# Haochen-Wang409/U2PL

Hardware: AMD Instinct MI355X
Metric: train images/sec at 769x769 (R101-DeepLabv3+) (higher is better)
Workload: dtype f32

## Files before the change

### include/u2pl_hip.h

```cpp
#ifndef U2PL_HIP_H
#define U2PL_HIP_H

#include <stddef.h>
#include <stdint.h>

#ifdef __cplusplus
extern "C" {
#endif

#ifndef __HIP_PLATFORM_AMD__
typedef struct ihipStream_t* hipStream_t;
#endif

#define U2PL_SEL_MAX_SLOTS 8
#define U2PL_SEL_WORD_NVALID 0
#define U2PL_SEL_WORD_NTOTAL 1
#define U2PL_SEL_WORD_VAL 40
#define U2PL_SEL_WORD_THR 56

int u2pl_bilinear_up_f32(const float* in, long sn, long sc, long sh, long sw, int N, int C, int h, int w,
                         float* out_nchw, int H, int W, hipStream_t stream);
int u2pl_bilinear_up_bwd_f32(const float* gout_nchw, int N, int C, int H, int W, float* gin, long sn, long sc,
                             long sh, long sw, int h, int w, hipStream_t stream);
int u2pl_pseudo_label_f32(const float* logits_nchw, int N, int C, int H, int W, float* conf, long long* label,
                          hipStream_t stream);
int u2pl_entropy_f32(const float* logits_nchw, const long long* label, int ignore, int N, int C, int H, int W,
                     float* entropy, unsigned* ws, hipStream_t stream);
int u2pl_entropy_up_f32(const float* in, long sn, long sc, long sh, long sw, int N, int C, int h, int w, int H, int W,
                        const long long* label, int ignore, float* entropy, unsigned* ws, hipStream_t stream);
size_t u2pl_select_workspace_bytes(void);
int u2pl_select_f32(const float* values, long n, int nspec, const int* spec_kind_dev, const float* q32_dev,
                    const long long* kparam_dev, const float* fparam_dev, unsigned* ws, int hist0_done,
                    hipStream_t stream);
int u2pl_apply_drop_i64(const float* entropy, const unsigned* thr_bits, long long* target, int ignore, long n,
                        unsigned* nkept, hipStream_t stream);
int u2pl_reliability_masks(const float* entropy, const unsigned* thr_lo_bits, const unsigned* thr_hi_bits,
                           const long long* label_l, const long long* label_u, int ignore, int B, int H, int W,
                           int h, int w, int negative_high_entropy, float* low_mask, float* high_mask,
                           unsigned* lbits, hipStream_t stream);
int u2pl_reliability_apply(const float* entropy, const unsigned* thr_bits, const long long* label_l,
                           const long long* label_u, int ignore, int B, int H, int W, int h, int w,
                           int negative_high_entropy, long long* target_u, unsigned* nkept, float* low_mask,
                           float* high_mask, unsigned* lbits, hipStream_t stream);
int u2pl_pack_class_bits(const long long* onehot, int N, int C, int h, int w, unsigned* bits, hipStream_t stream);
int u2pl_unpack_class_bits(const unsigned* bits, int N, int C, int h, int w, long long* onehot,
                           hipStream_t stream);

int u2pl_contra_classify(const float* prob, long sn, long sc, long sp, const unsigned* lbits,
                         const float* low_mask, const float* high_mask, int N2, int num_labeled, int C, int h,
                         int w, float thr_p, float thr_n, int low_rank, int high_rank, unsigned* abits,
                         unsigned* lowbits, unsigned* nbits, void* compact_workspace, hipStream_t stream);
size_t u2pl_compact_workspace_bytes(long P);
int u2pl_compact_lists(const unsigned* abits, const unsigned* lowbits, const unsigned* nbits, long P, int C,
                       void* workspace, int* idx, long cap, unsigned* counts, int counted, hipStream_t stream);
size_t u2pl_proto_workspace_bytes(long P, int C, int D);
int u2pl_class_prototypes(const float* rows, long ld, int D, const int* idx, long cap, const unsigned* counts,
                          int C, long P, void* workspace, float* proto, const unsigned* lowbits,
                          hipStream_t stream);
size_t u2pl_contra_phase1_workspace_bytes(long P, int C, int D);
int u2pl_contra_phase1(const float* prob, long sn, long sc, long sp, const unsigned* lbits, const float* low_mask,
                       const float* high_mask, int N2, int num_labeled, int C, int h, int w, float thr_p, float thr_n,
                       int low_rank, int high_rank, const float* rows, long ld, int D, unsigned* abits, unsigned* lowbits,
                       unsigned* nbits, int* idx, long cap, unsigned* counts, float* proto, void* workspace,
                       hipStream_t stream);
int u2pl_gather_rows_f32(const float* rows, long ld, int D, const int* list, long n, float* out,
                         hipStream_t stream);
size_t u2pl_bank_state_bytes(int C);
int u2pl_bank_init(long long* state, int C, const long long* caps_host, hipStream_t stream);
int u2pl_bank_enqueue_f32(long long* state, float* storage, int D, const float* rows, long ld, const int* idx,
                          long idx_stride, const long long* row_start_dev, const unsigned* counts_dev, int C,
                          hipStream_t stream);
int u2pl_bank_append_f32(float* bank, long cap, long tail, int D, const float* rows, long ld, const int* list,
                         long n_new, hipStream_t stream);
int u2pl_bank_append_multi_f32(const long long* desc_dev, int nclass, int D, long ld, long max_new,
                               hipStream_t stream);
size_t u2pl_infonce_job_bytes(void);
int u2pl_infonce_f32(const void* jobs_dev, int njobs, const float* rep, long ld, int D, int Q, int K,
                     float temp, float* loss_q, float* ganchor, int* anchor_pix, int* head, int* next,
                     const int* seg_len, hipStream_t stream);
size_t u2pl_infonce_fused_workspace_bytes(int njobs, int Q);
int u2pl_infonce_fused_f32(const void* jobs_dev, int njobs, const float* rep, long ld, int D, int Q, int K, float temp,
                           float* loss_q, float* ganchor, int* anchor_pix, int* head, int* next, const int* seg_len,
                           float* zero_dst, long zero_ld, const int* zero_pix, long zero_n, void* workspace,
                           float inv_valid_seg, float* loss, hipStream_t stream);
int u2pl_infonce_reduce_f32(const float* loss_q, int njobs, int Q, float inv_valid_seg, float* loss,
                            hipStream_t stream);
int u2pl_scatter_rows_ordered_f32(float* dst, long ld, int D, const int* pix, const int* next, int* head,
                                  const int* order, const int* seg_pos, const int* seg_len, const float* src, long n,
                                  const float* gout_dev, float scale, hipStream_t stream);
int u2pl_zero_rows_f32(float* dst, long ld, int D, const int* pix, long n, hipStream_t stream);

size_t u2pl_ce_workspace_bytes(void);
int u2pl_ce_fwd_f32(const float* logits_nchw, const long long* target, int ignore, int N, int C, int H, int W,
                    int unsup_weight, void* workspace, float* out3, hipStream_t stream);
int u2pl_ce_bwd_f32(const float* logits_nchw, const long long* target, int ignore, int N, int C, int H, int W,
                    const float* out3_dev, const float* gout_dev, float gmul, float* grad, hipStream_t stream);
int u2pl_ce_fwd_weighted_f32(const float* logits_nchw, const long long* target, int ignore, int N, int C, int H, int W,
                             const float* class_weight, void* workspace, float* out3, hipStream_t stream);
int u2pl_ce_bwd_weighted_f32(const float* logits_nchw, const long long* target, int ignore, int N, int C, int H, int W,
                             const float* class_weight, const float* out3_dev, const float* gout_dev, float gmul,
                             float* grad, hipStream_t stream);
int u2pl_ohem_prob_f32(const float* logits_nchw, const long long* target, int ignore, int N, int C, int H,
                       int W, float* mask_prob, unsigned* ws, hipStream_t stream);
int u2pl_ohem_apply_i64(const float* mask_prob, const unsigned* thr_bits, const long long* target, int ignore,
                        long n, long long* kept_target, hipStream_t stream);
int u2pl_confusion_hist_f32(const float* logits_nchw, const long long* target, int ignore, int N, int C, int H, int W,
                            long long* hist3c, hipStream_t stream);

int u2pl_predict_map_f32(const float* in, long sn, long sc, long sh, long sw, int N, int C, int h, int w, int H, int W,
                         unsigned char* label, const unsigned char* palette, unsigned char* rgb, hipStream_t stream);
int u2pl_infer_input_u8_f32(const unsigned char* img_hwc, int h, int w, const float* lut, float* out_hwc, int H, int W,
                            hipStream_t stream);
int u2pl_window_fuse_f32(float* pred, float* count, int C, int H, int W, const float* in, long sc, long sh, long sw, int h,
                         int w, int h0, int w0, int hc, int wc, int flip, int softmax, float weight, int bump,
                         hipStream_t stream);
int u2pl_predict_entropy_f32(const float* in, long sn, long sc, long sh, long sw, int N, int C, int h, int w, int H, int W,
                             int prob, unsigned char* label, float* entropy, hipStream_t stream);
int u2pl_reliable_map_u8(unsigned char* label, const float* entropy, const unsigned* thr_bits, long n,
                         const unsigned char* palette, unsigned char* rgb, unsigned char* heat, float heat_scale,
                         unsigned* ndropped, hipStream_t stream);
int u2pl_lut_u8(const unsigned char* in, unsigned char* out, long n, const unsigned char* lut256, hipStream_t stream);

int u2pl_conv2d_fwd_f32(const float* x, long ldx, const float* w, const float* bias, float* y, long ldy, int N,
                        int Hin, int Win, int Cin, int Hout, int Wout, int Cout, int R, int S, int stride,
                        int pad, int dil, hipStream_t stream);
int u2pl_conv2d_fwd_stat_blocks(int N, int Hout, int Wout, int Cout);
int u2pl_conv2d_fwd_bnstats_f32(const float* x, long ldx, const float* w, const float* bias, float* y, long ldy,
                                int N, int Hin, int Win, int Cin, int Hout, int Wout, int Cout, int R, int S,
                                int stride, int pad, int dil, const float* pivot, float* stats_partial,
                                hipStream_t stream);
int u2pl_colreduce_finish_f32(const float* partial, int nblk, int C, double* sums, hipStream_t stream);
int u2pl_conv2d_fwd_bnact_f32(const float* x, long ldx, const float* w, const float* bias, float* y, long ldy, int N,
                              int Hin, int Win, int Cin, int Hout, int Wout, int Cout, int R, int S, int stride,
                              int pad, int dil, const float* mean, const float* invstd, const float* gamma,
                              const float* beta, const float* res, long ldr, int relu, hipStream_t stream);
int u2pl_gemm_batched_f32(const float* x, long ldx, long zx, const float* w, long zw, float* y, long ldy, long zy,
                          long M, int K, int Nn, int batch, hipStream_t stream);
size_t u2pl_wino_tiles(int N, int H, int W, int dil, int mt);
int u2pl_wino_stat_blocks(long tiles, int O);
int u2pl_wino_input_f32(const float* x, long ldx, int N, int H, int W, int C, int dil, int mt, float* V,
                        hipStream_t stream);
int u2pl_wino_weight_f32(const float* w, int O, int C, int transposed, int mt, float* U, hipStream_t stream);
int u2pl_wino_gy_f32(const float* gy, long ldg, int N, int H, int W, int O, int dil, int mt, float* Mg,
                     hipStream_t stream);
int u2pl_wgrad_batched_splits(long M, int Cin, int Cout, int batch);
size_t u2pl_wgrad_batched_workspace_bytes(long M, int Cin, int Cout, int batch);
int u2pl_wgrad_batched_f32(const float* dy, long lddy, long zdy, const float* x, long ldx, long zx, float* part,
                           long M, int Cin, int Cout, int batch, hipStream_t stream);
int u2pl_wino_wgrad_finish_f32(const float* part, int nsplit, int O, int C, int mt, int accumulate, float* dw,
                               hipStream_t stream);
int u2pl_wino_output_f32(const float* Mb, int N, int H, int W, int O, int dil, int mt, const float* bias, float* y,
                         long ldy, float* stats_partial, const float* pivot, hipStream_t stream);
int u2pl_wino_output_bnact_f32(const float* Mb, int N, int H, int W, int O, int dil, int mt, const float* bias, float* y,
                               long ldy, const float* mean, const float* invstd, const float* gamma, const float* beta,
                               const float* res, long ldr, int relu, hipStream_t stream);
int u2pl_conv2d_fwd_bf16op_f32(const float* x, long ldx, const float* w, const float* bias, float* y, long ldy, int N,
                               int Hin, int Win, int Cin, int Hout, int Wout, int Cout, int R, int S, int stride,
                               int pad, int dil, hipStream_t stream);
int u2pl_conv2d_fwd_bnstats_bf16op_f32(const float* x, long ldx, const float* w, const float* bias, float* y, long ldy,
                                       int N, int Hin, int Win, int Cin, int Hout, int Wout, int Cout, int R, int S,
                                       int stride, int pad, int dil, const float* pivot, float* stats_partial,
                                       hipStream_t stream);
int u2pl_conv2d_dgrad_bf16op_f32(const float* dy, long lddy, const float* wT, float* dx, long lddx, int N, int Hin,
                                 int Win, int Cin, int Hout, int Wout, int Cout, int R, int S, int stride, int pad,
                                 int dil, hipStream_t stream);
int u2pl_conv2d_wgrad_bf16op_f32(const float* dy, long lddy, const float* x, long ldx, float* dw, void* workspace,
                                 int accumulate, int N, int Hin, int Win, int Cin, int Hout, int Wout, int Cout, int R,
                                 int S, int stride, int pad, int dil, hipStream_t stream);
int u2pl_conv2d_dgrad_f32(const float* dy, long lddy, const float* wT, float* dx, long lddx, int N, int Hin,
                          int Win, int Cin, int Hout, int Wout, int Cout, int R, int S, int stride, int pad,
                          int dil, hipStream_t stream);
int u2pl_weight_transpose_f32(const float* w, float* wt, int Cout, int RS, int Cin, hipStream_t stream);
size_t u2pl_conv2d_wgrad_workspace_bytes(int N, int Hout, int Wout, int Cin, int Cout, int R, int S);
int u2pl_conv2d_wgrad_f32(const float* dy, long lddy, const float* x, long ldx, float* dw, void* workspace,
                          int accumulate, int N, int Hin, int Win, int Cin, int Hout, int Wout, int Cout, int R,
                          int S, int stride, int pad, int dil, hipStream_t stream);
int u2pl_wgrad_set_tr(int on);
int u2pl_im2col_f32(const float* x, long ldx, float* col, int Kp, int N, int Hin, int Win, int Cin, int Hout,
                    int Wout, int R, int S, int stride, int pad, int dil, hipStream_t stream);

int u2pl_gconv2d_fwd_f32(const float* x, long ldx, const float* w, const float* bias, float* y, long ldy, int N, int Hin,
                         int Win, int Cin, int Hout, int Wout, int Cout, int R, int S, int stride, int pad, int dil,
                         int groups, hipStream_t stream);
int u2pl_gconv2d_dgrad_f32(const float* dy, long lddy, const float* w, float* dx, long lddx, int N, int Hin, int Win,
                           int Cin, int Hout, int Wout, int Cout, int R, int S, int stride, int pad, int dil, int groups,
                           hipStream_t stream);
size_t u2pl_gconv2d_wgrad_workspace_bytes(int N, int Hout, int Wout, int Cin, int Cout, int R, int S, int groups);
int u2pl_gconv2d_wgrad_f32(const float* dy, long lddy, const float* x, long ldx, float* dw, void* workspace,
                           int accumulate, int N, int Hin, int Win, int Cin, int Hout, int Wout, int Cout, int R,
                           int S, int stride, int pad, int dil, int groups, hipStream_t stream);

int u2pl_dwconv2d_fwd_f32(const float* x, long ldx, const float* w, const float* bias, float* y, long ldy, int N, int Hin,
                          int Win, int Cin, int Hout, int Wout, int Cout, int R, int S, int stride, int pad, int dil,
                          int groups, hipStream_t stream);
int u2pl_dwconv2d_dgrad_f32(const float* dy, long lddy, const float* w, float* dx, long lddx, int N, int Hin, int Win,
                            int Cin, int Hout, int Wout, int Cout, int R, int S, int stride, int pad, int dil, int groups,
                            hipStream_t stream);
size_t u2pl_dwconv2d_wgrad_workspace_bytes(int N, int Hout, int Wout, int Cin, int Cout, int R, int S, int groups);
int u2pl_dwconv2d_wgrad_f32(const float* dy, long lddy, const float* x, long ldx, float* dw, void* workspace,
                            int accumulate, int N, int Hin, int Win, int Cin, int Hout, int Wout, int Cout, int R,
                            int S, int stride, int pad, int dil, int groups, hipStream_t stream);

size_t u2pl_weight_split3_bytes(int rows, int K, int batch);
int u2pl_weight_split3_f32(const float* w, long zw, int rows, int K, int batch, void* out, hipStream_t stream);
int u2pl_weight_split3_multi_f32(const void* jobs, int njobs, long total, hipStream_t stream);
int u2pl_weight_split3_pad_rows(int rows);
int u2pl_wino_weight_multi_f32(const void* jobs, int njobs, long total, hipStream_t stream);
size_t u2pl_weight_split2h_bytes(int rows, int K, int batch);
int u2pl_weight_split2h_f32(const float* w, long zw, int rows, int K, int batch, void* out, hipStream_t stream);
int u2pl_weight_rebuild2h_job_bytes(void);
int u2pl_weight_rebuild2h_span(int which);
int u2pl_weight_rebuild2h_f32(const void* jobs, int n_flat, int n_wino, long seg_total, long amax_total, int wino_mblocks,
                              int wino_pblocks, hipStream_t stream);
int u2pl_amax_words(void);
int u2pl_absmax_f32(const float* x, long ld, long M, int C, float* out, int clear, hipStream_t stream);

int u2pl_igemm_ws_stat_blocks(int N, int Hout, int Wout);
int u2pl_igemm_ws_set_persist(int on);
int u2pl_conv2d_fwd_ws_f32(const float* x, long ldx, const void* wsplit, const float* bias, float* y, long ldy, int N,
                           int Hin, int Win, int Cin, int Hout, int Wout, int Cout, int R, int S, int stride, int pad,
                           int dil, hipStream_t stream);
int u2pl_conv2d_fwd_bnstats_ws_f32(const float* x, long ldx, const void* wsplit, const float* bias, float* y, long ldy,
                                   int N, int Hin, int Win, int Cin, int Hout, int Wout, int Cout, int R, int S,
                                   int stride, int pad, int dil, const float* pivot, float* stats_partial,
                                   hipStream_t stream);
int u2pl_conv2d_fwd_bnact_ws_f32(const float* x, long ldx, const void* wsplit, const float* bias, float* y, long ldy, int N,
                                 int Hin, int Win, int Cin, int Hout, int Wout, int Cout, int R, int S, int stride,
                                 int pad, int dil, const float* mean, const float* invstd, const float* gamma,
                                 const float* beta, const float* res, long ldr, int relu, hipStream_t stream);
int u2pl_conv2d_dgrad_ws_f32(const float* dy, long lddy, const void* wTsplit, float* dx, long lddx, int N, int Hin,
                             int Win, int Cin, int Hout, int Wout, int Cout, int R, int S, int stride, int pad, int dil,
                             hipStream_t stream);
int u2pl_gemm_batched_ws_f32(const float* x, long ldx, long zx, const void* wsplit, float* y, long ldy, long zy, long M,
                             int K, int Nn, int batch, hipStream_t stream);

int u2pl_bn_apply_amax_f32(const float* x, long ldx, const float* mean, const float* invstd, const float* gamma, const float* beta,
                           const float* res, long ldr, int relu, const float* drop, long rows_per_image, float* y, long ldy, long M,
                           int C, float* y_amax, hipStream_t stream);
int u2pl_bn_bwd_apply_amax_f32(const float* dy, long lddy, const float* x, long ldx, const float* y, long ldy, const float* mean,
                               const float* invstd, const float* gamma, const float* drop, long rows_per_image, const double* sums,
                               double count, float* dx, long lddx, float* dres, long lddr, long M, int C, const double* psums,
                               float* gsink, float* bsink, int accumulate, float* dx_amax, float* dres_amax, const float* relu_beta,
                               hipStream_t stream);
int u2pl_bn_bwd_sums_mx_f32(const float* dy, long lddy, const float* x, long ldx, const float* mean, const float* invstd,
                            const float* gamma, const float* beta, const float* drop, long rows_per_image, long M, int C,
                            void* workspace, double* sums, hipStream_t stream);
int u2pl_bn_apply_bits_f32(const float* x, long ldx, const float* mean, const float* invstd, const float* gamma, const float* beta,
                           const float* res, long ldr, int relu, const float* drop, long rows_per_image, float* y, long ldy, long M,
                           int C, float* y_amax, unsigned* bits, long ldb, hipStream_t stream);
int u2pl_bn_bwd_sums_bits_f32(const float* dy, long lddy, const float* x, long ldx, const unsigned* bits, long ldb,
                              const float* mean, const float* invstd, const float* drop, long rows_per_image, long M, int C,
                              void* workspace, double* sums, hipStream_t stream);
int u2pl_bn_bwd_apply_bits_f32(const float* dy, long lddy, const float* x, long ldx, const unsigned* bits, long ldb,
                               const float* mean, const float* invstd, const float* gamma, const float* drop, long rows_per_image,
                               const double* sums, double count, float* dx, long lddx, float* dres, long lddr, long M, int C,
                               const double* psums, float* gsink, float* bsink, int accumulate, float* dx_amax, float* dres_amax,
                               hipStream_t stream);
int u2pl_wino_input_amax_f32(const float* x, long ldx, int N, int H, int W, int C, int dil, int mt, float* V, float* v_amax,
                             hipStream_t stream);
int u2pl_wino_output_bnact_amax_f32(const float* Mb, int N, int H, int W, int O, int dil, int mt, const float* bias, float* y,
                                    long ldy, const float* mean, const float* invstd, const float* gamma, const float* beta,
                                    const float* res, long ldr, int relu, float* y_amax, hipStream_t stream);
int u2pl_wino_gy_amax_f32(const float* gy, long ldg, int N, int H, int W, int O, int dil, int mt, float* Mg, float* mg_amax,
                          hipStream_t stream);
int u2pl_conv2d_fwd_wsh_f32(const float* x, long ldx, const float* x_amax, const void* wsplit, const float* bias, float* y, long ldy,
                            int N, int Hin, int Win, int Cin, int Hout, int Wout, int Cout, int R, int S, int stride, int pad,
                            int dil, hipStream_t stream);
int u2pl_conv2d_fwd_bnstats_wsh_f32(const float* x, long ldx, const float* x_amax, const void* wsplit, const float* bias, float* y,
                                    long ldy, int N, int Hin, int Win, int Cin, int Hout, int Wout, int Cout, int R, int S,
                                    int stride, int pad, int dil, const float* pivot, float* stats_partial, hipStream_t stream);
int u2pl_conv2d_fwd_bnact_wsh_f32(const float* x, long ldx, const float* x_amax, const void* wsplit, const float* bias, float* y,
                                  long ldy, int N, int Hin, int Win, int Cin, int Hout, int Wout, int Cout, int R, int S,
                                  int stride, int pad, int dil, const float* mean, const float* invstd, const float* gamma,
                                  const float* beta, const float* res, long ldr, int relu, float* y_amax, hipStream_t stream);
int u2pl_conv2d_dgrad_wsh_f32(const float* dy, long lddy, const float* dy_amax, const void* wTsplit, float* dx, long lddx, int N,
                              int Hin, int Win, int Cin, int Hout, int Wout, int Cout, int R, int S, int stride, int pad, int dil,
                              hipStream_t stream);
int u2pl_gemm_batched_wsh_f32(const float* x, long ldx, long zx, const float* x_amax, const void* wsplit, float* y, long ldy, long zy,
                              long M, int K, int Nn, int batch, hipStream_t stream);
int u2pl_wgrad_h_eligible(int Cin, int Cout);
int u2pl_conv2d_wgrad_h_f32(const float* dy, long lddy, const float* dy_amax, const float* x, long ldx, const float* x_amax, float* dw,
                            void* workspace, int accumulate, int N, int Hin, int Win, int Cin, int Hout, int Wout, int Cout, int R,
                            int S, int stride, int pad, int dil, hipStream_t stream);
int u2pl_wgrad_batched_h_f32(const float* dy, long lddy, long zdy, const float* dy_amax, const float* x, long ldx, long zx,
                             const float* x_amax, float* part, long M, int Cin, int Cout, int batch, hipStream_t stream);

size_t u2pl_colreduce_workspace_bytes(long Mseg, int nseg, int C);
int u2pl_bn_stats_f32(const float* x, long ld, long M, int C, const float* pivot, void* workspace, double* sums,
                      hipStream_t stream);
int u2pl_colsum_f32(const float* x, long ld, long Mseg, int nseg, int C, void* workspace, double* sums,
                    hipStream_t stream);
int u2pl_bn_bwd_sums_f32(const float* dy, long lddy, const float* x, long ldx, const float* y, long ldy,
                         const float* mean, const float* invstd, const float* drop, long rows_per_image, long M,
                         int C, void* workspace, double* sums, hipStream_t stream);
int u2pl_bn_finalize_f32(const double* sums, double count, const float* pivot, int C, float eps, float momentum,
                         float* mean, float* invstd, float* running_mean, float* running_var, hipStream_t stream);
int u2pl_bn_eval_invstd_f32(const float* running_var, int C, float eps, float* invstd, hipStream_t stream);
int u2pl_bn_finish_finalize_f32(const float* partial, int nblk, int C, double count, const float* pivot, float eps,
                                float momentum, float* mean, float* invstd, float* running_mean, float* running_var,
                                double* sums_out, hipStream_t stream);
size_t u2pl_bn_eval_invstd_job_bytes(void);
int u2pl_bn_eval_invstd_multi_f32(const void* jobs_dev, int njobs, long total, hipStream_t stream);
int u2pl_bn_apply_f32(const float* x, long ldx, const float* mean, const float* invstd, const float* gamma,
                      const float* beta, const float* res, long ldr, int relu, const float* drop,
                      long rows_per_image, float* y, long ldy, long M, int C, hipStream_t stream);
int u2pl_bn_bwd_apply_f32(const float* dy, long lddy, const float* x, long ldx, const float* y, long ldy,
                          const float* mean, const float* invstd, const float* gamma, const float* drop,
                          long rows_per_image, const double* sums, double count, float* dx, long lddx, float* dres,
                          long lddr, long M, int C, hipStream_t stream);
int u2pl_bn_bwd_apply_pg_f32(const float* dy, long lddy, const float* x, long ldx, const float* y, long ldy,
                             const float* mean, const float* invstd, const float* gamma, const float* drop,
                             long rows_per_image, const double* sums, double count, float* dx, long lddx, float* dres,
                             long lddr, long M, int C, const double* psums, float* gsink, float* bsink, int accumulate,
                             hipStream_t stream);
int u2pl_sums_to_f32(const double* sums, int n, float scale, int accumulate, float* out, hipStream_t stream);
int u2pl_maxpool3s2_fwd_f32(const float* x, long ldx, int N, int H, int W, int C, int Ho, int Wo, float* y, long ldy,
                            unsigned char* tap, hipStream_t stream);
int u2pl_maxpool3s2_bwd_f32(const float* dy, long lddy, const unsigned char* tap, int N, int H, int W, int C, int Ho,
                            int Wo, float* dx, long lddx, hipStream_t stream);
int u2pl_copy_rows_f32(const float* src, long lds, float* dst, long ldd, long M, int C, int accumulate,
                       hipStream_t stream);
int u2pl_copy_cols_f32(const float* src, long lds, float* dst, long ldd, long M, int C, hipStream_t stream);
int u2pl_broadcast_rows_f32(const float* v, long ldv, float scale, float* dst, long ldd, long rows_per_image, long M,
                            int C, hipStream_t stream);
int u2pl_bilinear_rows_fwd_f32(const float* x, long ldx, int N, int h, int w, int C, int H, int W, float* y, long ldy,
                               hipStream_t stream);
int u2pl_bilinear_rows_bwd_f32(const float* dy, long lddy, int N, int h, int w, int C, int H, int W, float* dx,
                               long lddx, hipStream_t stream);
int u2pl_softmax_rows_f32(const float* x, long ldx, float* y, long ldy, long M, int C, hipStream_t stream);
int u2pl_sgd_step_f32(float* p, const float* g, float* buf, long n, long b1, long b2, float lr0, float lr1, float lr2,
                      float momentum, float weight_decay, int first, float grad_scale, hipStream_t stream);
int u2pl_ema_update_f32(float* t, const float* s, long n, float decay, float one_minus_decay, hipStream_t stream);
int u2pl_adam_step_f32(float* p, const float* g, float* exp_avg, float* exp_avg_sq, long n, long b1, long b2, float lr0,
                       float lr1, float lr2, float beta1, float one_minus_beta1, float beta2, float one_minus_beta2,
                       float eps, float weight_decay, float bias_correction1, float bias_correction2_sqrt,
                       float grad_scale, hipStream_t stream);
size_t u2pl_kernel_launches(void);
int u2pl_conv_set_split(int on);
int u2pl_conv_get_split(void);
int u2pl_debug_phase1_times(unsigned* buf);
size_t u2pl_reliability_fused_workspace_bytes(int G);
size_t u2pl_reliability_fused_cand_floats(long n_px, int G);
int u2pl_reliability_fused(const float* logits_low, long sn, long sc, long sh, long sw, int B, int C, int h, int w,
                           int H, int W, const long long* label_u, const long long* label_l, int ignore, int nspec,
                           const float* q32_host, int negative_high_entropy, int hm, int wm, float* entropy,
                           long long* target_u, float* low_mask, float* high_mask, unsigned* lbits,
                           unsigned* workspace, float* cand, int G, unsigned epoch, int flags, hipStream_t stream);
int u2pl_cutmix_f32(const float* img, const long long* label, const float* conf, const int* boxes_dev, int B, int C,
                    int H, int W, float* out_img, long long* out_label, float* out_conf, hipStream_t stream);

int u2pl_dense_small_f32(const float* x, long ldx, const float* w, const float* bias, float* y, long ldy, int M, int K,
                         int Cout, hipStream_t stream);
int u2pl_strong_aug_f32(const float* img, const long long* label, const float* conf, const int* boxes_dev,
                        const unsigned long long* sel_dev, int mode, int B, int C, int H, int W, float* out_img,
                        long long* out_label, float* out_conf, hipStream_t stream);
int u2pl_label_presence_i64(const long long* label, int B, long HW, unsigned long long* bits, hipStream_t stream);

int u2pl_window_accumulate_f32(float* pred, float* count, int C, int H, int W, const float* src, int h0, int w0,
                               int hc, int wc, hipStream_t stream);
int u2pl_window_normalize_f32(float* pred, const float* count, int C, int H, int W, hipStream_t stream);

int u2pl_augment_u8_f32(const unsigned char* img, const unsigned char* lab, const int* params, int B, int H, int W,
                        int Sh, int Sw, const float* mean3, const float* std3, float* out_img, long long* out_lab,
                        hipStream_t stream);

#define U2PL_AUG_REC 16
#define U2PL_AUG_ROTATE 1
#define U2PL_AUG_BLUR 2
size_t u2pl_augment_ex_scratch_bytes(int B, int Sh, int Sw, int mode);
int u2pl_augment_ex_u8_f32(const unsigned char* img, const unsigned char* lab, const long long* offsets,
                           const int* records, int B, int H, int W, int Sh, int Sw, int ignore_label, int mode,
                           const float* mean3, const float* std3, const float* blur_w, float* scratch, float* out_img,
                           long long* out_lab, hipStream_t stream);
int u2pl_augment_lut_u8_f32(const unsigned char* img, const unsigned char* lab, const long long* offsets,
                            const int* records, int B, int H, int W, int Sh, int Sw, int ignore_label, int mode,
                            const unsigned char* lut256, const float* mean3, const float* std3, const float* blur_w,
                            float* scratch, float* out_img, long long* out_lab, hipStream_t stream);

int u2pl_half_weight_f16(const float* w, int Cout, int Cin, int R, int S, unsigned short* out, hipStream_t stream);
int u2pl_hconv2d_fwd_f16(const unsigned short* x, long ldx, const unsigned short* w, const float* scale,
                         const float* shift, const unsigned short* res, long ldr, void* y, long ldy, int N, int Hin,
                         int Win, int Cin, int Hout, int Wout, int Cout, int R, int S, int stride, int pad, int dil,
                         int relu, int out_f32, int tile, int* sat, hipStream_t stream);
int u2pl_hconv2d_stem_f16(const float* x, long ldx, const unsigned short* w, const float* scale, const float* shift,
                          unsigned short* y, long ldy, int N, int Hin, int Win, int Cin, int Hout, int Wout, int Cout,
                          int R, int S, int stride, int pad, int dil, int relu, int* sat, hipStream_t stream);
int u2pl_hmaxpool3s2_f16(const unsigned short* x, long ldx, int N, int H, int W, int C, int Ho, int Wo,
                         unsigned short* y, long ldy, hipStream_t stream);
int u2pl_hgap_f16(const unsigned short* x, long ldx, int N, int HW, int C, unsigned short* y, hipStream_t stream);
int u2pl_hbilinear_f16(const unsigned short* x, long ldx, int N, int h, int w, int C, unsigned short* y, long ldy,
                       int H, int W, hipStream_t stream);

int u2pl_wide_words(int C);
int u2pl_reliability_masks_wide(const float* entropy, const unsigned* thr_lo_bits, const unsigned* thr_hi_bits,
                                const long long* label_l, const long long* label_u, int ignore, int B, int H, int W,
                                int h, int w, int negative_high_entropy, int C, float* low_mask, float* high_mask,
                                unsigned* lbits, hipStream_t stream);
int u2pl_reliability_apply_wide(const float* entropy, const unsigned* thr_bits, const long long* label_l,
                                const long long* label_u, int ignore, int B, int H, int W, int h, int w,
                                int negative_high_entropy, int C, long long* target_u, unsigned* nkept, float* low_mask,
                                float* high_mask, unsigned* lbits, hipStream_t stream);
int u2pl_pack_class_bits_wide(const long long* onehot, int N, int C, int h, int w, unsigned* bits, hipStream_t stream);
int u2pl_unpack_class_bits_wide(const unsigned* bits, int N, int C, int h, int w, long long* onehot, hipStream_t stream);
size_t u2pl_contra_wide_workspace_bytes(long P, int C);
int u2pl_contra_wide_block_pixels(int C);
int u2pl_contra_wide_staged(int C);
int u2pl_contra_classify_wide(const float* prob, long sn, long sc, long sp, const unsigned* lbits, const float* low_mask,
                              const float* high_mask, int N2, int num_labeled, int C, int h, int w, float thr_p,
                              float thr_n, int low_rank, int high_rank, unsigned* abits, unsigned* lowbits,
                              unsigned* nbits, void* workspace, unsigned* counts, long long* offsets,
                              hipStream_t stream);
int u2pl_compact_lists_wide(const unsigned* abits, const unsigned* lowbits, const unsigned* nbits, long P, int C,
                            const void* workspace, const long long* offsets, int* idx, long idx_len,
                            hipStream_t stream);
int u2pl_class_prototypes_wide(const float* rows, long ld, int D, const int* idx, const long long* offsets,
                               const unsigned* counts, int C, float* proto, hipStream_t stream);
int u2pl_bank_init_wide(long long* state, int C, const long long* caps_host, hipStream_t stream);
int u2pl_bank_enqueue_wide_f32(long long* state, float* storage, int D, const float* rows, long ld, const int* idx,
                               const long long* list_off_dev, const long long* row_start_dev,
                               const unsigned* counts_dev, int C, hipStream_t stream);

#ifdef __cplusplus
}
#endif
#endif
```

### u2pl_amd/csrc/wgrad_tr.h

```cpp
#pragma once
#include "conv_geom.h"

bool wgrad_tr_eligible(const ConvGeom& g);
void wgrad_tr_plan(const ConvGeom& g, int taps, int& ctiles, int& nsplit, int& cps);
int launch_wgrad_tr(const float* dy, long lddy, const float* x, long ldx, float* part, const ConvGeom& g, int ctiles, int nsplit,
                    int cps, hipStream_t stream, long zdy, long zx, const float* dy_amax = nullptr, const float* x_amax = nullptr);
```

### u2pl_amd/csrc/wgrad_tr.hip

```cpp
#include <stdlib.h>
#include <type_traits>
#include "common.h"
#include "conv_geom.h"
#include "u2pl_hip.h"
#include "wgrad_tr.h"

template <int B, int E, class F>
__device__ __forceinline__ void wt_static_for(F&& f) {
    if constexpr (B < E) {
        f(std::integral_constant<int, B>{});
        wt_static_for<B + 1, E>(f);
    }
}
typedef short v4s16 __attribute__((ext_vector_type(4)));
typedef short v8s16 __attribute__((ext_vector_type(8)));
#define WT_LDS(p) ((__attribute__((address_space(3))) v4s16*)(p))

template <int TN, bool PW, int NP = 3>
__global__ __launch_bounds__(512, 2) void k_wgrad_tr(const float* __restrict__ dy, long lddy, const float* __restrict__ x,
                                                     long ldx, float* __restrict__ part, ConvGeom g, int ctiles,
                                                     int chunks_per_split, unsigned dybytes, unsigned xbytes, long zdy,
                                                     long zx, const float* __restrict__ dy_amax, const float* __restrict__ x_amax) {
    constexpr int TM = 2, WN = 4, BM = 128, BN = 32 * TN * WN, CH = BM + BN;
    constexpr int PITCH = CH * 2 + 64;
    constexpr int PL = BK * PITCH, ST = NP * PL;
    constexpr int NLA = BM / 64, NLB = BN / 64, NLD = NLA + NLB;
    constexpr int NPROD = NP == 3 ? 6 : 3;
    constexpr int PER = TM * TN, NMF = 2 * NPROD * PER, NRD = NP * (TM + TN) * 2;
    int e_dy = 0, e_x = 0;
    float s_dy = 1.f, s_x = 1.f;
    if constexpr (NP == 2) {
        e_dy = split2_exp_bits(amax_read((const unsigned*)dy_amax));
        e_x = split2_exp_bits(amax_read((const unsigned*)x_amax));
        s_dy = split2_scale(e_dy);
        s_x = split2_scale(e_x);
    }
    using C0 = std::integral_constant<int, 0>;
    using C1 = std::integral_constant<int, 1>;
    {
        const int tap_b = blockIdx.x / ctiles;
        dy += (long)tap_b * zdy;
        x += (long)tap_b * zx;
    }
    const __amdgpu_buffer_rsrc_t rdy = make_rsrc(dy, dybytes), rx = make_rsrc(x, xbytes);
    extern __shared__ __attribute__((aligned(16))) unsigned char smem[];
    const int tid = threadIdx.x, lane = tid & 63, wave = tid >> 6;
    const int wm = wave / WN, wn = wave % WN;
    const long M = (long)g.N * g.Hout * g.Wout;
    const int co0 = blockIdx.y * BM;
    const int tap = blockIdx.x / ctiles, ci0 = (blockIdx.x - tap * ctiles) * BN;
    const int tr = tap / g.S, ts_ = tap - tr * g.S;
    const long nchunks = (M + BK - 1) / BK;
    const long c_begin = (long)blockIdx.z * chunks_per_split;
    const int nk = (int)(min(nchunks, c_begin + chunks_per_split) - c_begin);

    const int px = tid >> 4, q = tid & 15;
    const int lddyb = (int)lddy * 4, ldxb = (int)ldx * 4;
    float4 r[2][NLD];
    int l_kc = 0;
    auto load_one = [&](auto set_c, auto i_c, int dyo, int xo) __attribute__((always_inline)) {
        constexpr int SET = decltype(set_c)::value, i = decltype(i_c)::value;
        if constexpr (i < NLA) {
            const int co = co0 + 4 * (q + 16 * i);
            r[SET][i] = buf_load4(rdy, (dyo != OOB_OFF && co < g.Cout) ? dyo + co * 4 : OOB_OFF);
        } else {
            const int ci = ci0 + 4 * (q + 16 * (i - NLA));
            r[SET][i] = buf_load4(rx, (xo != OOB_OFF && ci < g.Cin) ? xo + ci * 4 : OOB_OFF);
        }
    };
    auto row_offsets = [&](int& dyo, int& xo) __attribute__((always_inline)) {
        const long m = (c_begin + l_kc) * BK + px;
        const bool mv = m < M;
        const unsigned mm = mv ? (unsigned)m : 0u;
        dyo = mv ? (int)mm * lddyb : OOB_OFF;
        if constexpr (PW) {
            xo = mv ? (int)mm * ldxb : OOB_OFF;
        } else {
            const unsigned t = mm / (unsigned)g.Wout;
            const int wo = (int)(mm - t * (unsigned)g.Wout);
            const unsigned n_ = t / (unsigned)g.Hout;
            const int ho = (int)(t - n_ * (unsigned)g.Hout);
            int ih, iw;
            const bool okh = gather_coord(ho * g.mul + g.off_h, tr, g.step, 0, g.Hin, ih);
            const bool okw = gather_coord(wo * g.mul + g.off_w, ts_, g.step, 0, g.Win, iw);
            xo = (mv & okh & okw) ? ((int)n_ * g.Hin * g.Win + ih * g.Win + iw) * ldxb : OOB_OFF;
        }
    };
    auto load_all = [&](auto set_c) __attribute__((always_inline)) {
        int dyo, xo;
        row_offsets(dyo, xo);
        wt_static_for<0, NLD>([&](auto i) __attribute__((always_inline)) { load_one(set_c, i, dyo, xo); });
        l_kc = min(l_kc + 1, nk - 1);
    };
    auto st_off = [&](int i) __attribute__((always_inline)) {
        const int ch = i < NLA ? 4 * (q + 16 * i) : BM + 4 * (q + 16 * (i - NLA));
        return px * PITCH + ch * 2;
    };
    auto store_f4 = [&](int stage, int i, uint2 p0, uint2 p1, uint2 p2) __attribute__((always_inline)) {
        unsigned char* d = smem + stage * ST + st_off(i);
        *(uint2*)d = p0;
        *(uint2*)(d + PL) = p1;
        if constexpr (NP == 3) *(uint2*)(d + 2 * PL) = p2;
    };

    f32x16 acc[TM][TN];
#pragma unroll
    for (int a = 0; a < TM; ++a)
#pragma unroll
        for (int b = 0; b < TN; ++b)
#pragma unroll
            for (int e = 0; e < 16; ++e) acc[a][b][e] = 0.f;

    const int li = lane & 31, lh = lane >> 5, lj = lane & 15, lblk = (lane >> 4) & 1;
    const int lbase = (8 * lh + (lj >> 2)) * PITCH + (16 * lblk + 4 * (lj & 3)) * 2;
    const int afr = lbase + (wm * 64) * 2, bfr = lbase + (BM + wn * 32 * TN) * 2;
    struct Frag { v4s16 a[NP][TM][2], b[NP][TN][2]; };
    Frag f[2];
    auto do_read = [&](auto stage_c, auto gk_c, auto j_c) __attribute__((always_inline)) {
        constexpr int stage = decltype(stage_c)::value, gk = decltype(gk_c)::value, J = decltype(j_c)::value;
        if constexpr (J < NRD) {
            constexpr int h = J & 1, F = J >> 1, qq = F / (TM + TN), w = F % (TM + TN);
            constexpr int rowoff = (16 * gk + 4 * h) * PITCH;
            if constexpr (w < TM)
                f[gk].a[NP - 1 - qq][w][h] = __builtin_amdgcn_ds_read_tr16_b64_v4i16(WT_LDS(smem + stage * ST + (NP - 1 - qq) * PL + rowoff + w * 64 + afr));
            else
                f[gk].b[qq][w - TM][h] = __builtin_amdgcn_ds_read_tr16_b64_v4i16(WT_LDS(smem + stage * ST + qq * PL + rowoff + (w - TM) * 64 + bfr));
        }
    };
    using frag_t = std::conditional_t<NP == 3, bf16x8, f16x8>;
    auto frag8 = [&](const v4s16 (&hh)[2]) __attribute__((always_inline)) {
        v8s16 v = __builtin_shufflevector(hh[0], hh[1], 0, 1, 2, 3, 4, 5, 6, 7);
        return __builtin_bit_cast(frag_t, v);
    };
    auto do_mfma = [&](auto i_c) __attribute__((always_inline)) {
        constexpr int I = decltype(i_c)::value;
        constexpr int PA[6] = {2, 1, 0, 1, 0, 0}, PB[6] = {0, 1, 2, 0, 1, 0};
        constexpr int QA[3] = {1, 0, 0}, QB[3] = {0, 1, 0};
        constexpr int gk = I / (NPROD * PER), qq = (I / PER) % NPROD, ab = I % PER, a = ab / TN, b = ab % TN;
        if constexpr (NP == 3) acc[a][b] = __builtin_amdgcn_mfma_f32_32x32x16_bf16(frag8(f[gk].a[PA[qq]][a]), frag8(f[gk].b[PB[qq]][b]), acc[a][b], 0, 0, 0);
        else acc[a][b] = __builtin_amdgcn_mfma_f32_32x32x16_f16(frag8(f[gk].a[QA[qq]][a]), frag8(f[gk].b[QB[qq]][b]), acc[a][b], 0, 0, 0);
    };

    load_all(C0{});
#pragma unroll
    for (int i = 0; i < NLD; ++i) {
        uint2 p0, p1, p2 = make_uint2(0, 0);
        if constexpr (NP == 3) split3_bf16(r[0][i], p0, p1, p2);
        else split2_f16(r[0][i], i < NLA ? s_dy : s_x, p0, p1);
        store_f4(0, i, p0, p1, p2);
    }
    __builtin_amdgcn_sched_barrier(0);
    load_all(C1{});
    __builtin_amdgcn_sched_barrier(0);
    load_all(C0{});
    __builtin_amdgcn_sched_barrier(0);
    __syncthreads();
#pragma unroll
    for (int p = 0; p < NP; ++p) {
#pragma unroll
        for (int h = 0; h < 2; ++h) {
#pragma unroll
            for (int a = 0; a < TM; ++a) f[1].a[p][a][h] = (v4s16){0, 0, 0, 0};
#pragma unroll
            for (int b = 0; b < TN; ++b) f[1].b[p][b][h] = (v4s16){0, 0, 0, 0};
        }
    }

    uint2 pc[3];
    float sp_l = 0.f, sp_h = 0.f;
    int n_dyo = 0, n_xo = 0;
    auto chunk = [&](auto par_c) __attribute__((always_inline)) {
        constexpr int cur = decltype(par_c)::value, nxt = cur ^ 1;
        using CUR = std::integral_constant<int, cur>;
        using NXT = std::integral_constant<int, nxt>;
        constexpr int TAIL = 2 * PER;
        constexpr int F0_PRE = 2 * (TM + TN), F0_PER = (NRD - F0_PRE + TAIL - 1) / TAIL;
        constexpr int LD_SLOTS = (NLD + 1) / 2;
        constexpr int SP_START = NP == 3 ? TAIL : 0;
        constexpr int SPP = NP == 3 ? ((NMF - TAIL - LD_SLOTS) / (2 * NLD) >= 3 ? 3 : 2) : ((NMF - LD_SLOTS) / (2 * NLD) >= 2 ? 2 : 1);
        constexpr int F1_START = TAIL, F1_PER = (NRD + NPROD * PER - 1) / (NPROD * PER);
        constexpr int SP_END = SP_START + SPP * 2 * NLD, LD_START = SP_END;
        static_assert(F1_START + (NRD + F1_PER - 1) / F1_PER <= TAIL + NPROD * PER, "k block 1 operands would be read after their first use");
        static_assert(LD_START + LD_SLOTS <= NMF, "split + loads do not fit the chunk");
        wt_static_for<0, F0_PRE>([&](auto j) __attribute__((always_inline)) { do_read(CUR{}, C0{}, j); });
        __builtin_amdgcn_sched_barrier(0);
        wt_static_for<0, NMF>([&](auto sl_c) __attribute__((always_inline)) {
            constexpr int sl = decltype(sl_c)::value;
            do_mfma(std::integral_constant<int, (sl < TAIL ? NMF - TAIL + sl : sl - TAIL)>{});
            if constexpr (sl < TAIL)
                wt_static_for<0, F0_PER>([&](auto u) __attribute__((always_inline)) { do_read(CUR{}, C0{}, std::integral_constant<int, F0_PRE + sl * F0_PER + decltype(u)::value>{}); });
            if constexpr (sl >= F1_START)
                wt_static_for<0, F1_PER>([&](auto u) __attribute__((always_inline)) { do_read(CUR{}, C1{}, std::integral_constant<int, (sl - F1_START) * F1_PER + decltype(u)::value>{}); });
            if constexpr (sl >= SP_START && sl < SP_END) {
                constexpr int k = (sl - SP_START) / SPP, s_in = (sl - SP_START) % SPP;
                constexpr int st0 = NP == 3 ? (SPP == 3 ? s_in : (s_in == 0 ? 0 : 2)) : (SPP == 2 ? s_in : 0);
                constexpr int st1 = NP == 3 ? (SPP == 3 ? s_in : (s_in == 0 ? 1 : 2)) : (SPP == 2 ? s_in : 1);
                wt_static_for<st0, st1 + 1>([&](auto step_c) __attribute__((always_inline)) {
                    constexpr int step = decltype(step_c)::value;
                    if constexpr (step == 0) {
                        const float4 v = r[nxt][k >> 1];
                        sp_l = (k & 1) ? v.z : v.x;
                        sp_h = (k & 1) ? v.w : v.y;
                    }
                    unsigned w;
                    if constexpr (NP == 2) {
                        const float sc = (k >> 1) < NLA ? s_dy : s_x;
                        if constexpr (step == 0) w = split2_first(sp_l, sp_h, sc);
                        else w = split2_second(sp_l, sp_h, sc, (k & 1) ? pc[0].y : pc[0].x);
                    } else {
                        w = step == 0 ? pack2_bf16_first(sp_l, sp_h) : pack2_bf16(sp_l, sp_h);
                        if constexpr (step < 2) {
                            sp_l = sp_l - bf16_lo_f(w);
                            sp_h = sp_h - bf16_hi_f(w);
                        }
                    }
                    if constexpr (k & 1) pc[step].y = w; else pc[step].x = w;
                    if constexpr ((k & 1) && step == NP - 1) store_f4(nxt, k >> 1, pc[0], pc[1], pc[NP - 1]);
                });
            }
            if constexpr (sl == LD_START - 1) row_offsets(n_dyo, n_xo);
            if constexpr (sl >= LD_START && sl < LD_START + LD_SLOTS) {
                constexpr int i0 = 2 * (sl - LD_START);
                load_one(NXT{}, std::integral_constant<int, i0>{}, n_dyo, n_xo);
                if constexpr (i0 + 1 < NLD) load_one(NXT{}, std::integral_constant<int, i0 + 1>{}, n_dyo, n_xo);
                if constexpr (sl == LD_START + LD_SLOTS - 1) l_kc = min(l_kc + 1, nk - 1);
            }
            __builtin_amdgcn_sched_barrier(0);
        });
        __syncthreads();
    };
    {
        int kc = 0;
        for (; kc + 1 < nk; kc += 2) {
            chunk(C0{});
            chunk(C1{});
        }
        if (kc < nk) chunk(C0{});
        wt_static_for<0, 2 * PER>([&](auto sl) __attribute__((always_inline)) { do_mfma(std::integral_constant<int, NMF - 2 * PER + decltype(sl)::value>{}); });
    }

    const long wsz = (long)g.Cout * g.R * g.S * g.Cin;
    float* out = part + (long)blockIdx.z * wsz;
    const long rowlen = (long)g.R * g.S * g.Cin;
#pragma unroll
    for (int a = 0; a < TM; ++a)
#pragma unroll
        for (int b = 0; b < TN; ++b) {
            const int ci = ci0 + wn * 32 * TN + b * 32 + li;
            if (ci >= g.Cin) continue;
#pragma unroll
            for (int e = 0; e < 16; ++e) {
                const int co = co0 + wm * 64 + a * 32 + (e & 3) + 8 * (e >> 2) + 4 * lh;
                if (co < g.Cout) out[(long)co * rowlen + (long)tap * g.Cin + ci] = NP == 2 ? __builtin_ldexpf(acc[a][b][e], -(e_dy + e_x)) : acc[a][b][e];
            }
        }
}

static int g_wgrad_tr = -1;
static int wgrad_tr_on() {
    if (g_wgrad_tr < 0) { const char* e = getenv("U2PL_WGRAD_TR"); g_wgrad_tr = (e && *e) ? (atoi(e) != 0) : 1; }
    return g_wgrad_tr;
}
U2PL_API int u2pl_wgrad_set_tr(int on) { const int old = wgrad_tr_on(); g_wgrad_tr = on != 0; return old; }
bool wgrad_tr_eligible(const ConvGeom& g) {
    return wgrad_tr_on() && g.Cout >= 128 && g.Cin >= 128 && !(g.Cout % 4) && !(g.Cin % 4);
}
static int wt_bn(const ConvGeom& g) {
    static int force = -1;
    if (force < 0) { const char* e = getenv("U2PL_WT_BN"); force = (e && *e) ? atoi(e) : 0; }
    if (force == 128 || force == 256) return force;
    return g.Cin > 128 ? 256 : 128;
}
void wgrad_tr_plan(const ConvGeom& g, int taps, int& ctiles, int& nsplit, int& cps) {
    const long M = (long)g.N * g.Hout * g.Wout;
    const long nchunks = (M + BK - 1) / BK;
    ctiles = cdiv(g.Cin, wt_bn(g));
    const long tiles = (long)cdiv(g.Cout, 128) * ctiles * taps;
    long best = 1;
    double bestc = 1e30;
    const long maxs = nchunks / 6 > 0 ? nchunks / 6 : 1;
    for (long s = 1; s <= maxs && s <= 96; ++s) {
        const long c = (nchunks + s - 1) / s;
        if ((nchunks + c - 1) / c != s) continue;
        const double rounds = (double)cdiv(tiles * s, 256);
        const double cost = rounds * (c + 5.0) + 0.15 * s;
        if (cost < bestc) { bestc = cost; best = s; }
    }
    cps = (int)((nchunks + best - 1) / best);
    nsplit = (int)((nchunks + cps - 1) / cps);
}

template <int TN, bool PW, int NP>
static int launch1(const float* dy, long lddy, const float* x, long ldx, float* part, const ConvGeom& g, int ctiles, int nsplit,
                   int cps, int taps, hipStream_t stream, long zdy, long zx, const float* dy_amax, const float* x_amax) {
    constexpr int CH = 128 + 128 * TN, PITCH = CH * 2 + 64;
    const size_t lds = (size_t)2 * NP * BK * PITCH;
    static bool attr_set = false;
    if (!attr_set) {
        (void)hipFuncSetAttribute((const void*)k_wgrad_tr<TN, PW, NP>, hipFuncAttributeMaxDynamicSharedMemorySize, (int)lds);
        attr_set = true;
    }
    const long dyb = (((long)g.N * g.Hout * g.Wout - 1) * lddy + g.Cout) * 4;
    const long xb = (((long)g.N * g.Hin * g.Win - 1) * ldx + g.Cin) * 4;
    if (dyb >= (1L << 31) || xb >= (1L << 31)) return U2PL_EINVAL;
    dim3 grid((unsigned)(ctiles * taps), (unsigned)cdiv(g.Cout, 128), (unsigned)nsplit);
    U2PL_LAUNCH((k_wgrad_tr<TN, PW, NP>), grid, dim3(512), lds, stream, dy, lddy, x, ldx, part, g, ctiles, cps, (unsigned)dyb,
                (unsigned)xb, zdy, zx, dy_amax, x_amax);
    U2PL_LAUNCH_CHECK();
    return 0;
}
template <int NP>
static int launch_np(const float* dy, long lddy, const float* x, long ldx, float* part, const ConvGeom& g, int ctiles, int nsplit,
                     int cps, hipStream_t stream, long zdy, long zx, const float* dy_amax, const float* x_amax) {
    const int taps = g.R * g.S;
    const bool pw = g.mul == 1 && g.off_h == 0 && g.off_w == 0 && g.Hin == g.Hout && g.Win == g.Wout && (g.step == 0 || taps == 1);
    if (wt_bn(g) == 256)
        return pw ? launch1<2, true, NP>(dy, lddy, x, ldx, part, g, ctiles, nsplit, cps, taps, stream, zdy, zx, dy_amax, x_amax)
                  : launch1<2, false, NP>(dy, lddy, x, ldx, part, g, ctiles, nsplit, cps, taps, stream, zdy, zx, dy_amax, x_amax);
    return pw ? launch1<1, true, NP>(dy, lddy, x, ldx, part, g, ctiles, nsplit, cps, taps, stream, zdy, zx, dy_amax, x_amax)
              : launch1<1, false, NP>(dy, lddy, x, ldx, part, g, ctiles, nsplit, cps, taps, stream, zdy, zx, dy_amax, x_amax);
}
int launch_wgrad_tr(const float* dy, long lddy, const float* x, long ldx, float* part, const ConvGeom& g, int ctiles, int nsplit,
                    int cps, hipStream_t stream, long zdy, long zx, const float* dy_amax, const float* x_amax) {
    if ((dy_amax == nullptr) != (x_amax == nullptr)) return U2PL_EINVAL;
    return dy_amax ? launch_np<2>(dy, lddy, x, ldx, part, g, ctiles, nsplit, cps, stream, zdy, zx, dy_amax, x_amax)
                   : launch_np<3>(dy, lddy, x, ldx, part, g, ctiles, nsplit, cps, stream, zdy, zx, nullptr, nullptr);
}
```

Before: 37.82.

## Remap wgrad block IDs so XCD-resident blocks share input tiles in L2

Flattens the wgrad grid to one dimension and remaps block IDs with a swizzle. Blocks dispatched round-robin to the same XCD (id mod 8) then cover a small group of Cout tiles, Cin tiles and taps that reuse the same dy/x slices. The supergroup shape is chosen to minimise loaded bytes per block, up to 32 blocks. The aim is to cut L2 misses and HBM traffic on MI355X's multi-XCD layout, at the cost of some integer index math per block and a new env toggle.

Result: no change. 38.13 (median of 6 runs) (+0.8%).

```diff
diff --git a/include/u2pl_hip.h b/include/u2pl_hip.h
--- a/include/u2pl_hip.h
+++ b/include/u2pl_hip.h
@@ -176,6 +176,9 @@
                           int accumulate, int N, int Hin, int Win, int Cin, int Hout, int Wout, int Cout, int R,
                           int S, int stride, int pad, int dil, hipStream_t stream);
 int u2pl_wgrad_set_tr(int on);
+int u2pl_wgrad_set_xcd_map(int on);
+int u2pl_wgrad_tr_block_map(int gx, int gy, int gz, int id, int* out);
+int u2pl_wgrad_tr_block_map_all(int ctiles, int taps, int batch, int gy, int gz, int bn, int* out, int* sub);
 int u2pl_im2col_f32(const float* x, long ldx, float* col, int Kp, int N, int Hin, int Win, int Cin, int Hout,
                     int Wout, int R, int S, int stride, int pad, int dil, hipStream_t stream);
 
diff --git a/u2pl_amd/csrc/wgrad_tr.h b/u2pl_amd/csrc/wgrad_tr.h
--- a/u2pl_amd/csrc/wgrad_tr.h
+++ b/u2pl_amd/csrc/wgrad_tr.h
@@ -5,3 +5,35 @@
 void wgrad_tr_plan(const ConvGeom& g, int taps, int& ctiles, int& nsplit, int& cps);
 int launch_wgrad_tr(const float* dy, long lddy, const float* x, long ldx, float* part, const ConvGeom& g, int ctiles, int nsplit,
                     int cps, hipStream_t stream, long zdy, long zx, const float* dy_amax = nullptr, const float* x_amax = nullptr);
+
+struct WtBlockMap {
+    int gx, gy, gz, ctiles;
+    int sy, sc, st;
+};
+__host__ __device__ inline void wt_block_map(const WtBlockMap& m, unsigned id, int& x, int& y, int& z) {
+    if (m.sy == 0) {
+        x = (int)(id % (unsigned)m.gx);
+        const unsigned t = id / (unsigned)m.gx;
+        y = (int)(t % (unsigned)m.gy);
+        z = (int)(t / (unsigned)m.gy);
+        return;
+    }
+    const unsigned S = (unsigned)(m.sy * m.sc * m.st), n = (unsigned)m.gx * m.gy * m.gz;
+    const unsigned head = n / (8u * S) * (8u * S);
+    unsigned p;
+    if (id < head) {
+        const unsigned l = id & 7u, k = id >> 3;
+        p = ((k / S) * 8u + l) * S + k % S;
+    } else {
+        const unsigned t = id - head, l = t & 7u, k = t >> 3, mm = n - head, q = mm >> 3, r = mm & 7u;
+        p = head + (l < r ? l * (q + 1u) : r * (q + 1u) + (l - r) * q) + k;
+    }
+    const unsigned j = p / S, w = p % S;
+    const unsigned ny = (unsigned)(m.gy / m.sy), nc = (unsigned)(m.ctiles / m.sc), nt = (unsigned)(m.gx / m.ctiles / m.st);
+    const unsigned t_in = w % (unsigned)m.st, c_in = (w / (unsigned)m.st) % (unsigned)m.sc, y_in = w / (unsigned)(m.st * m.sc);
+    const unsigned yb = j % ny, cb = (j / ny) % nc, tb = (j / (ny * nc)) % nt;
+    z = (int)(j / (ny * nc * nt));
+    x = (int)((tb * m.st + t_in) * m.ctiles + cb * m.sc + c_in);
+    y = (int)(yb * m.sy + y_in);
+}
+WtBlockMap wgrad_tr_block_map(int ctiles, int taps, bool batch, int gy, int gz, int bn);
diff --git a/u2pl_amd/csrc/wgrad_tr.hip b/u2pl_amd/csrc/wgrad_tr.hip
--- a/u2pl_amd/csrc/wgrad_tr.hip
+++ b/u2pl_amd/csrc/wgrad_tr.hip
@@ -18,7 +18,7 @@
 
 template <int TN, bool PW, int NP = 3>
 __global__ __launch_bounds__(512, 2) void k_wgrad_tr(const float* __restrict__ dy, long lddy, const float* __restrict__ x,
-                                                     long ldx, float* __restrict__ part, ConvGeom g, int ctiles,
+                                                     long ldx, float* __restrict__ part, ConvGeom g, WtBlockMap bm,
                                                      int chunks_per_split, unsigned dybytes, unsigned xbytes, long zdy,
                                                      long zx, const float* __restrict__ dy_amax, const float* __restrict__ x_amax) {
     constexpr int TM = 2, WN = 4, BM = 128, BN = 32 * TN * WN, CH = BM + BN;
@@ -37,8 +37,11 @@
     }
     using C0 = std::integral_constant<int, 0>;
     using C1 = std::integral_constant<int, 1>;
+    const int ctiles = bm.ctiles;
+    int bx, by, bz;
+    wt_block_map(bm, blockIdx.x, bx, by, bz);
     {
-        const int tap_b = blockIdx.x / ctiles;
+        const int tap_b = bx / ctiles;
         dy += (long)tap_b * zdy;
         x += (long)tap_b * zx;
     }
@@ -47,11 +50,11 @@
     const int tid = threadIdx.x, lane = tid & 63, wave = tid >> 6;
     const int wm = wave / WN, wn = wave % WN;
     const long M = (long)g.N * g.Hout * g.Wout;
-    const int co0 = blockIdx.y * BM;
-    const int tap = blockIdx.x / ctiles, ci0 = (blockIdx.x - tap * ctiles) * BN;
+    const int co0 = by * BM;
+    const int tap = bx / ctiles, ci0 = (bx - tap * ctiles) * BN;
     const int tr = tap / g.S, ts_ = tap - tr * g.S;
     const long nchunks = (M + BK - 1) / BK;
-    const long c_begin = (long)blockIdx.z * chunks_per_split;
+    const long c_begin = (long)bz * chunks_per_split;
     const int nk = (int)(min(nchunks, c_begin + chunks_per_split) - c_begin);
 
     const int px = tid >> 4, q = tid & 15;
@@ -240,7 +243,7 @@
     }
 
     const long wsz = (long)g.Cout * g.R * g.S * g.Cin;
-    float* out = part + (long)blockIdx.z * wsz;
+    float* out = part + (long)bz * wsz;
     const long rowlen = (long)g.R * g.S * g.Cin;
 #pragma unroll
     for (int a = 0; a < TM; ++a)
@@ -264,6 +267,45 @@
 U2PL_API int u2pl_wgrad_set_tr(int on) { const int old = wgrad_tr_on(); g_wgrad_tr = on != 0; return old; }
 bool wgrad_tr_eligible(const ConvGeom& g) {
     return wgrad_tr_on() && g.Cout >= 128 && g.Cin >= 128 && !(g.Cout % 4) && !(g.Cin % 4);
+}
+static int g_wgrad_xcd = -1;
+static int wgrad_xcd_on() {
+    if (g_wgrad_xcd < 0) { const char* e = getenv("U2PL_WGRAD_XCD"); g_wgrad_xcd = (e && *e) ? (atoi(e) != 0) : 1; }
+    return g_wgrad_xcd;
+}
+U2PL_API int u2pl_wgrad_set_xcd_map(int on) { const int old = wgrad_xcd_on(); g_wgrad_xcd = on != 0; return old; }
+WtBlockMap wgrad_tr_block_map(int ctiles, int taps, bool batch, int gy, int gz, int bn) {
+    WtBlockMap m = {ctiles * taps, gy, gz, ctiles, 0, 0, 0};
+    if (!wgrad_xcd_on()) return m;
+    const int gt = batch ? 1 : taps;
+    long bc = 0, bs = 0;
+    for (int sy = 1; sy <= gy && sy <= 32; ++sy) {
+        if (gy % sy) continue;
+        for (int sc = 1; sc <= ctiles && sy * sc <= 32; ++sc) {
+            if (ctiles % sc) continue;
+            for (int st = 1; st <= gt && sy * sc * st <= 32; ++st) {
+                if (gt % st) continue;
+                const long c = 128L * sy + (long)bn * sc, s = (long)sy * sc * st;
+                if (bs == 0 || c * bs < bc * s || (c * bs == bc * s && s > bs)) { bc = c; bs = s; m.sy = sy; m.sc = sc; m.st = st; }
+            }
+        }
+    }
+    return m;
+}
+U2PL_API int u2pl_wgrad_tr_block_map_all(int ctiles, int taps, int batch, int gy, int gz, int bn, int* out, int* sub) {
+    if (ctiles < 1 || taps < 1 || gy < 1 || gz < 1 || (bn != 128 && bn != 256) || !out) return U2PL_EINVAL;
+    if ((long)ctiles * taps * gy * gz >= (1L << 31)) return U2PL_EINVAL;
+    const WtBlockMap m = wgrad_tr_block_map(ctiles, taps, batch != 0, gy, gz, bn);
+    const unsigned n = (unsigned)m.gx * gy * gz;
+    for (unsigned id = 0; id < n; ++id) wt_block_map(m, id, out[3 * id], out[3 * id + 1], out[3 * id + 2]);
+    if (sub) { sub[0] = m.sy; sub[1] = m.sc; sub[2] = m.st; }
+    return 0;
+}
+U2PL_API int u2pl_wgrad_tr_block_map(int gx, int gy, int gz, int id, int* out) {
+    if (gx < 1 || gy < 1 || gz < 1 || !out || id < 0 || (long)gx * gy * gz >= (1L << 31) || id >= (long)gx * gy * gz) return U2PL_EINVAL;
+    const WtBlockMap m = wgrad_tr_block_map(gx, 1, false, gy, gz, 256);
+    wt_block_map(m, (unsigned)id, out[0], out[1], out[2]);
+    return 0;
 }
 static int wt_bn(const ConvGeom& g) {
     static int force = -1;
@@ -303,8 +345,11 @@
     const long dyb = (((long)g.N * g.Hout * g.Wout - 1) * lddy + g.Cout) * 4;
     const long xb = (((long)g.N * g.Hin * g.Win - 1) * ldx + g.Cin) * 4;
     if (dyb >= (1L << 31) || xb >= (1L << 31)) return U2PL_EINVAL;
-    dim3 grid((unsigned)(ctiles * taps), (unsigned)cdiv(g.Cout, 128), (unsigned)nsplit);
-    U2PL_LAUNCH((k_wgrad_tr<TN, PW, NP>), grid, dim3(512), lds, stream, dy, lddy, x, ldx, part, g, ctiles, cps, (unsigned)dyb,
+    const int gy = cdiv(g.Cout, 128);
+    if ((long)ctiles * taps * gy * nsplit >= (1L << 31)) return U2PL_EINVAL;
+    const WtBlockMap bm = wgrad_tr_block_map(ctiles, taps, g.step == 0 && taps > 1, gy, nsplit, 128 * TN);
+    dim3 grid((unsigned)(bm.gx * bm.gy * bm.gz));
+    U2PL_LAUNCH((k_wgrad_tr<TN, PW, NP>), grid, dim3(512), lds, stream, dy, lddy, x, ldx, part, g, bm, cps, (unsigned)dyb,
                 (unsigned)xb, zdy, zx, dy_amax, x_amax);
     U2PL_LAUNCH_CHECK();
     return 0;
```
